# Zolkin1/bilevel-gait-gen

Measured on NVIDIA B200. Metric: A1 SRB-MPC RTI solves/sec, higher is better.
Workload: dtype f64

## Files before the change

bilevel-gait-gen_b200/csrc/bgg_chol.cuh:

```cuda
#pragma once
#include <cuda_runtime.h>

namespace bgg {
namespace chol {

#ifdef BGG_IPM_PROF
static __device__ long long g_chol_prof[16];
#define CPROF_DECL long long cprof_t = clock64();
#define CPROF(k) do { if (threadIdx.x == 0 && blockIdx.x == 0) { const long long t_ = clock64(); g_chol_prof[k] += t_ - cprof_t; cprof_t = t_; } } while (0)
#else
#define CPROF_DECL
#define CPROF(k) do { } while (0)
#endif

__device__ __forceinline__ int blk(int bi, int bj) { return (((bi * (bi + 1)) >> 1) + bj) << 6; }
__device__ __forceinline__ int at(int i, int j) { return blk(i >> 3, j >> 3) + ((i & 7) << 3) + (j & 7); }
__host__ __device__ inline size_t doubles(int nb) { return static_cast<size_t>(nb) * (nb + 1) / 2 * 64; }

__device__ __forceinline__ void dmma(double& c0, double& c1, double a, double b) {
#ifdef BGG_NO_DMMA
    c0 = fma(a, b, c0);
    return;
#endif
    asm volatile("mma.sync.aligned.m8n8k4.row.col.f64.f64.f64.f64 {%0,%1}, {%2}, {%3}, {%0,%1};" : "+d"(c0), "+d"(c1) : "d"(a), "d"(b));
// ... 86 lines not shown
            }
    }
    __syncwarp();
    return bad_any;
}

__device__ __forceinline__ bool factor_invert_diag_v0(double* D, int lane) {
    bool bad_any = false;
    if (lane == 0) {
        double a[8][8];
#pragma unroll
        for (int r = 0; r < 8; ++r)
#pragma unroll
            for (int c = 0; c <= r; ++c) a[r][c] = D[r * 8 + c];
#pragma unroll
        for (int c = 0; c < 8; ++c) {
            const double d = a[c][c];
            const bool bad = !(d > 0.0);
            bad_any |= bad;
            const double inv = bad ? 1.0 : fast_rsqrt(d);
            a[c][c] = inv;
#pragma unroll
            for (int r = c + 1; r < 8; ++r) a[r][c] *= inv;
#pragma unroll
            for (int c2 = c + 1; c2 < 8; ++c2)
#pragma unroll
                for (int r = c2; r < 8; ++r) a[r][c2] -= a[r][c] * a[c2][c];
        }
#pragma unroll
        for (int r = 0; r < 8; ++r)
#pragma unroll
            for (int c = 0; c <= r; ++c) D[r * 8 + c] = a[r][c];
    }
    __syncwarp();
    double x[8];
    if (lane < 8) {
#pragma unroll
        for (int r = 0; r < 8; ++r) {
            double s = 0.0;
#pragma unroll
            for (int k = 0; k < r; ++k) s += D[r * 8 + k] * x[k];
            const double ir = D[r * 8 + r];
            x[r] = (r == lane) ? ir : ((r < lane) ? 0.0 : -ir * s);
        }
    }
    __syncwarp();
    if (lane < 8) {
#pragma unroll
        for (int r = 0; r < 8; ++r) D[r * 8 + lane] = x[r];
    }
    return bad_any;
}

static __device__ __noinline__ void factor(double* K, int nb, int* flag) {
    __builtin_assume(__isShared(K));
    __builtin_assume(__isShared(flag));
    const int tid = threadIdx.x, lane = tid & 31, wid = tid >> 5, nwarp = blockDim.x >> 5;
    if (tid == 0) *flag = 0;
    __syncthreads();
    double2 keep = make_double2(0.0, 0.0);
    CPROF_DECL
    if (wid == 0 && factor_invert_diag(K + blk(0, 0), lane)) *flag = 1;
    __syncthreads();
    const int nother = (nwarp - 1) * 32;
    for (int j = 0; j + 1 < nb; ++j) {
        const double2 X = ldfrag(K + blk(j, j), lane);
        double2 Lj1 = make_double2(0.0, 0.0);
        mma_pqT(Lj1, ldfrag(K + blk(j + 1, j), lane), X);
        if (wid == 0) {
            if (j > 0) stfrag(K + blk(j, j - 1), lane, keep);
            keep = Lj1;
            double2 upd = make_double2(0.0, 0.0);
            mma_pqT(upd, Lj1, Lj1);
            double2 c = ldfrag(K + blk(j + 1, j + 1), lane);
            c.x -= upd.x;
            c.y -= upd.y;
            stfrag(K + blk(j + 1, j + 1), lane, c);
            __syncwarp();
            if (factor_invert_diag(K + blk(j + 1, j + 1), lane)) *flag = 1;
            CPROF(0);
        } else {
            for (int i = j + 2 + (wid - 1); i < nb; i += nwarp - 1) {
                double2 Lij = make_double2(0.0, 0.0);
                mma_pqT(Lij, ldfrag(K + blk(i, j), lane), X);
                stfrag(K + blk(i, j), lane, Lij);
                double2 upd = make_double2(0.0, 0.0);
                mma_pqT(upd, Lij, Lj1);
                double2 c = ldfrag(K + blk(i, j + 1), lane);
                c.x -= upd.x;
                c.y -= upd.y;
                stfrag(K + blk(i, j + 1), lane, c);
            }
            asm volatile("bar.sync 1, %0;" ::"r"(nother) : "memory");
            const int jc = j + 2;
            for (int i = jc + (wid - 1); i < nb; i += nwarp - 1) {
                double2 a0 = make_double2(0.0, 0.0), a1 = make_double2(0.0, 0.0);
                const double* Li = K + blk(i, 0);
                const double* Lj = K + blk(jc, 0);
                int k = 0;
                for (; k + 1 <= j; k += 2) {
                    const double2 p0 = ldfrag(Li + (k << 6), lane), q0 = ldfrag(Lj + (k << 6), lane);
                    const double2 p1 = ldfrag(Li + ((k + 1) << 6), lane), q1 = ldfrag(Lj + ((k + 1) << 6), lane);
                    mma_pqT(a0, p0, q0);
                    mma_pqT(a1, p1, q1);
                }
                if (k <= j) mma_pqT(a0, ldfrag(Li + (k << 6), lane), ldfrag(Lj + (k << 6), lane));
                double2 c = ldfrag(Li + (jc << 6), lane);
                c.x -= a0.x + a1.x;
                c.y -= a0.y + a1.y;
                stfrag(K + blk(i, jc), lane, c);
            }
        }
        __syncthreads();
        CPROF(1);
    }
    if (wid == 0 && nb > 1) stfrag(K + blk(nb - 1, nb - 2), lane, keep);
    __syncthreads();
    CPROF(4);
    for (int h = 1; h <= 4; h <<= 1) {
        const int ngroup = (nb + 2 * h - 1) / (2 * h);
        for (int it = wid; it < ngroup * h; it += nwarp) {
            const int q = it / h, b0 = 2 * h * q, r = b0 + h + it % h;
            if (r >= nb) continue;
            for (int c = b0; c < b0 + h; ++c) {
                double2 T = make_double2(0.0, 0.0);
                for (int k = c; k < b0 + h; ++k) mma_pqT(T, ldfrag(K + blk(r, k), lane), ldfragT(K + blk(k, c), lane));
                __syncwarp();
                stfrag(K + blk(r, c), lane, T);
            }
        }
        __syncthreads();
        for (int it = wid; it < ngroup * h; it += nwarp) {
            const int q = it / h, b0 = 2 * h * q, c = b0 + it % h;
            const int rtop = (b0 + 2 * h < nb) ? b0 + 2 * h : nb;
            for (int r = rtop - 1; r >= b0 + h; --r) {
                double2 Xn = make_double2(0.0, 0.0);
                for (int k = b0 + h; k <= r; ++k) mma_pqT(Xn, ldfrag(K + blk(r, k), lane), ldfragT(K + blk(k, c), lane));
                __syncwarp();
                stfrag(K + blk(r, c), lane, make_double2(-Xn.x, -Xn.y));
                __syncwarp();
            }
        }
        __syncthreads();
    }
    CPROF(5);
}

static __device__ __noinline__ void solve(const double* K, int nb, double* v, double* ys) {
    __builtin_assume(__isShared(K));
    __builtin_assume(__isShared(v));
    __builtin_assume(__isShared(ys));
    const int tid = threadIdx.x, lane = tid & 31, wid = tid >> 5, nwarp = blockDim.x >> 5;
    const int g = lane >> 2, t = lane & 3;
    const int nsup = (nb + 7) >> 3;
    auto row_dot = [&](const double* Kr, const double* x, int qlo, int qhi) -> double {
        double a0 = 0.0, a1 = 0.0;
#pragma unroll 1
        for (int q0 = qlo; q0 < qhi; q0 += 4) {
            double2 p[4], xx[4];
#pragma unroll
            for (int u = 0; u < 4; ++u)
                if (q0 + u < qhi) {
                    p[u] = ldfrag(Kr + ((q0 + u) << 6), lane);
                    xx[u] = *reinterpret_cast<const double2*>(x + 8 * (q0 + u) + 2 * t);
                }
#pragma unroll
            for (int u = 0; u < 4; ++u)
                if (q0 + u < qhi) {
                    a0 = fma(p[u].x, xx[u].x, a0);
                    a1 = fma(p[u].y, xx[u].y, a1);
                }
        }
        a0 += a1;
        a0 += __shfl_xor_sync(0xffffffffu, a0, 1);
        a0 += __shfl_xor_sync(0xffffffffu, a0, 2);
        return a0;
    };
    auto col_dot = [&](int rlo, int rhi, int c, const double* x, int xoff) -> double2 {
        double ax = 0.0, ay = 0.0;
#pragma unroll 1
        for (int r0 = rlo; r0 < rhi; r0 += 4) {
            double2 p[4];
            double xv[4];
#pragma unroll
            for (int u = 0; u < 4; ++u)
                if (r0 + u < rhi) {
                    p[u] = ldfrag(K + blk(r0 + u, c), lane);
                    xv[u] = x[8 * (r0 + u - xoff) + g];
                }
#pragma unroll
            for (int u = 0; u < 4; ++u)
                if (r0 + u < rhi) {
                    ax = fma(p[u].x, xv[u], ax);
                    ay = fma(p[u].y, xv[u], ay);
                }
        }
#pragma unroll
        for (int o = 4; o < 32; o <<= 1) {
            ax += __shfl_xor_sync(0xffffffffu, ax, o);
            ay += __shfl_xor_sync(0xffffffffu, ay, o);
        }
        return make_double2(ax, ay);
    };
    __syncthreads();
    for (int s = 0; s < nsup; ++s) {
        const int b0 = 8 * s, b1 = (b0 + 8 < nb) ? b0 + 8 : nb, cnt = b1 - b0;
        if (wid < cnt) {
            const double a = row_dot(K + blk(b0 + wid, 0), v, b0, b0 + wid + 1);
            if (t == 0) ys[8 * wid + g] = a;
        }
        __syncthreads();
        for (int i = b1 + wid; i < nb; i += nwarp) {
            const double a = row_dot(K + blk(i, 0), ys - 8 * b0, b0, b1);
            if (t == 0) v[8 * i + g] -= a;
        }
        if (tid < 8 * cnt) v[8 * b0 + tid] = ys[tid];
        __syncthreads();
    }
    for (int s = nsup - 1; s >= 0; --s) {
        const int b0 = 8 * s, b1 = (b0 + 8 < nb) ? b0 + 8 : nb, cnt = b1 - b0;
        if (wid < cnt) {
            const double2 a = col_dot(b0 + wid, b1, b0 + wid, v, 0);
            if (g == 0) *reinterpret_cast<double2*>(ys + 8 * wid + 2 * t) = a;
        }
        __syncthreads();
        for (int kb = wid; kb < b0; kb += nwarp) {
            const double2 a = col_dot(b0, b1, kb, ys, b0);
            if (g == 0) {
                double2* dst = reinterpret_cast<double2*>(v + 8 * kb + 2 * t);
                double2 cur = *dst;
                cur.x -= a.x;
                cur.y -= a.y;
                *dst = cur;
            }
        }
        if (tid < 8 * cnt) v[8 * b0 + tid] = ys[tid];
        __syncthreads();
    }
}

}
}
```

bilevel-gait-gen_b200/csrc/bgg_ipm.cu:

```cuda
#include <cstdio>
#include <cstdlib>

#include "bgg_kernels.cuh"
#include "bgg_chol.cuh"
#include "bgg_kkt.cuh"
#include "bgg_kkt_mma.cuh"
#include "bgg_l2ops.cuh"
#ifdef BGG_IPM_TRACE
#include "bgg_ipm_trace.cuh"
#endif

namespace bgg {

#ifdef BGG_IPM_PROF
__device__ long long g_ipm_prof[32];
#define PROF_DECL __shared__ long long s_prof[32]; long long prof_t = 0; if (threadIdx.x == 0) { for (int i_ = 0; i_ < 32; ++i_) s_prof[i_] = 0; prof_t = clock64(); }
#define PROF(k) do { if (threadIdx.x == 0) { const long long t_ = clock64(); s_prof[k] += t_ - prof_t; prof_t = t_; } } while (0)
#define PROF_DUMP do { if (threadIdx.x == 0 && blockIdx.x == 0) for (int i_ = 0; i_ < 32; ++i_) g_ipm_prof[i_] = s_prof[i_]; } while (0)
#else
#define PROF_DECL
#define PROF(k) do { } while (0)
#define PROF_DUMP do { } while (0)
#endif

// ... 55 lines not shown
            fv[cc] = s;
        }
        double* o = out + 6 * j;
        o[0] = fv[2];
        o[1] = -fv[2];
        o[2] = fv[0] - mu_f * fv[2];
        o[3] = -fv[0] - mu_f * fv[2];
        o[4] = fv[1] - mu_f * fv[2];
        o[5] = -fv[1] - mu_f * fv[2];
    }
    if (eout != nullptr && tid >= nth - 32 && tid - (nth - 32) < c.neq) {
        const EqRow& q = c.eq[tid - (nth - 32)];
        double s = -rhs_scale * q.rhs;
        for (int i = 0; i < q.cnt; ++i) s += q.w[i] * v[q.col[i]];
        eout[tid - (nth - 32)] = s;
    }
    __syncthreads();
    #pragma unroll 1
    for (int e = tid; e < ne; e += nth) {
        const int cc = e & 1, foot = (e >> 1) & 3, kk = e >> 3, kf = kk * 4 + foot;
        const double* vv = v + nf + pbase[foot] + cc * npv[foot] + S.poff[kf];
        double s = -S.tkc[kk * 2 + cc];
        for (int i = 0; i < S.pcnt[kf]; ++i) s += S.pw[2 * kf + i] * vv[i];
        out[6 * ns + 2 * e] = s;
        out[6 * ns + 2 * e + 1] = -s;
    }
    __syncthreads();
}

template <bool kRowsShared, int kThreads>
static __device__ __forceinline__ void ipm_add_Ct(const IpmCtx& c, const double* y, double* out, const double* ey, double escale) {
    const Smem S = c.S;
    if (kRowsShared) __builtin_assume(__isShared(y)); __builtin_assume(__isShared(out)); __builtin_assume(__isShared(S.ckc));
    __builtin_assume(__isShared(S.smp)); __builtin_assume(__isShared(S.pw)); __builtin_assume(__isShared(S.col));
    __builtin_assume(__isShared(S.poff));
    const int tid = threadIdx.x;
    constexpr int nth = kThreads;
    const int nu = c.nu, nf = c.nf, ns = c.ns, nkc = c.nkc;
    const double mu_f = c.mu_f;
    #pragma unroll 1
    for (int q = tid; q < nkc; q += nth) {
        const int kk = q >> 1, cc = q & 1;
        double s = 0;
        for (int foot = 0; foot < kNumEE; ++foot) {
            const int e = (kk * 4 + foot) * 2 + cc;
            s += y[6 * ns + 2 * e] - y[6 * ns + 2 * e + 1];
        }
        S.ckc[q] = -s;
    }
    __syncthreads();
    l2_phi_cols_dot(S.phi, S.phi_stride, nkc, nf, smem_addr(S.ckc), smem_addr(out));
    {
        const int half = (2 * nu <= nth) ? 2 : 1;
        #pragma unroll 1
        for (int base = 0; base < half * nu; base += nth) {
            const int it = base + tid;
            const bool act = it < half * nu;
            const int col = act ? it / half : 0, part = it % half;
            const ColInfo ci = S.col[col];
            double s = 0;
            if (!act) {
            } else if (col < nf) {
                if (part == 1 || half == 1)
                    #pragma unroll 1
                    for (int j = ci.lo; j < ci.hi; ++j) {
                        const Sample& sp = S.smp[j];
                        const double* yy = y + 6 * j;
                        double coef;
                        if (ci.coord == 2) coef = (yy[0] - yy[1]) - mu_f * (yy[2] + yy[3] + yy[4] + yy[5]);
                        else if (ci.coord == 0) coef = yy[2] - yy[3];
                        else coef = yy[4] - yy[5];
                        s += coef * sp.w[ci.var - sp.off];
                    }
            } else {
                const int mid = (half == 2) ? (ci.lo + ci.hi + 1) / 2 : ci.hi;
                const int k0 = (part == 0) ? ci.lo : mid, k1 = (part == 0) ? mid : ci.hi;
                #pragma unroll 1
                for (int kk = k0; kk < k1; ++kk) {
                    const int kf = kk * 4 + ci.foot, e = kf * 2 + ci.coord;
                    s += (y[6 * ns + 2 * e] - y[6 * ns + 2 * e + 1]) * S.pw[2 * kf + (ci.var - S.poff[kf])];
                }
                if (ey != nullptr && part == 0) {
                    double se = 0;
                    const int grp = ci.foot * 2 + ci.coord;
                    #pragma unroll 1
                    for (int r = 0; r < c.neq; ++r) {
                        const EqRow& q = c.eq[r];
                        if (q.pad != grp) continue;
                        for (int i = 0; i < q.cnt; ++i)
                            if (q.col[i] == col) se += ey[r] * q.w[i];
                    }
                    s += escale * se;
                }
            }
            if (half == 2) s += __shfl_xor_sync(0xffffffffu, s, 1);
            if (act && part == 0) out[col] += s;
        }
    }
    __syncthreads();
}

static __device__ __forceinline__ void ipm_apply_H(const IpmCtx& c, const double* v, double* out, bool subtract) {
    l2_apply_H(c.Hg, c.nu, smem_addr(v), smem_addr(out), subtract);
}

struct IpmCaps {
// ... 121 lines not shown
        S.poff[i] = nl.poff[foot];
        S.pw[2 * i] = nl.pw[foot][0];
        S.pw[2 * i + 1] = nl.pw[foot][1];
    }
    __shared__ int s_fbase[kNumEE], s_pbase[kNumEE], s_nfv[kNumEE], s_npv[kNumEE];
    __shared__ int s_flag, s_nitems, s_nwork, s_npos;
    __shared__ KktWork s_work[kMaxKktWork];
    __shared__ int s_sb[kNumEE + 1];
    __shared__ EqRow s_eq[kMaxEq];
    if (tid < neq) s_eq[tid] = eqs[tid];
    if (tid < kNumEE) {
        s_fbase[tid] = Hd->fbase[tid];
        s_pbase[tid] = Hd->pbase[tid];
        s_nfv[tid] = Hd->nfv[tid];
        s_npv[tid] = Hd->npv[tid];
    }
    #pragma unroll 1
    for (int i = tid; i < 6 * cap_nu; i += nth) S.u[i] = 0.0;
    if (tid == 0) {
        int e = 0;
        s_sb[0] = 0;
        for (int j = 0; j < ns; ++j)
            while (samples[j].ee > e) s_sb[++e] = j;
        while (e < kNumEE) s_sb[++e] = ns;
    }

    const double box0 = Hd->ee_box[0] / 2, box1 = Hd->ee_box[1] / 2;
    const double fbound = P.force_bound;
    const int m_force = 6 * ns;
    int m_act = 0;
    #pragma unroll 1
    for (int j = tid; j < ns; j += nth) {
        const bool act = samples[j].active != 0;
        for (int r = 0; r < 6; ++r) {
            S.lam[6 * j + r] = act ? 1.0 : 0.0;
            S.s[6 * j + r] = 1.0;
        }
        m_act += act ? 6 : 0;
    }
    #pragma unroll 1
    for (int e = tid; e < ne; e += nth) {
        const int c = e & 1, foot = (e >> 1) & 3, kk = e >> 3;
        const double bx = c ? box1 : box0;
        const double off = xoff[(kk + kEENodeStart) * kNx + c];
        S.d[2 * e + 0] = (bx + P.hip_xy[foot][c]) + off;
        S.d[2 * e + 1] = -(-bx + P.hip_xy[foot][c]) - off;
        S.lam[m_force + 2 * e + 0] = 1.0;
        S.lam[m_force + 2 * e + 1] = 1.0;
        S.s[m_force + 2 * e + 0] = 1.0;
        S.s[m_force + 2 * e + 1] = 1.0;
        m_act += 2;
    }
    auto rhs_of = [&](int i) -> double { return (i < m_force) ? ((i % 6 == 0) ? fbound : 0.0) : S.d[i - m_force]; };
    m_act = static_cast<int>(block_reduce<kSum>(static_cast<double>(m_act), S.red) + 0.5);
    kkt_build_colinfo(S.col, nu, nf, N, s_fbase, s_pbase, s_nfv, s_npv, s_sb, S.smp, S.pcnt, S.poff);
    __syncthreads();
    KktItem* kitems = reinterpret_cast<KktItem*>(ws + L.ktab);
    KktPos* kpos = reinterpret_cast<KktPos*>(ws + L.ktab + sizeof(KktItem) * kMaxKktItems);
    kkt_mma_setup(s_work, &s_nwork, (nu + 7) >> 3, kitems, &s_nitems, s_fbase, s_nfv, S.col, S.smp, kpos, &s_npos, nu, nf, s_eq, neq);
    if (s_nitems > kMaxKktItems || s_npos > kMaxKktPos) {
        if (tid == 0) {
            Hd->status = kOther;
            Hd->no_iterate = 1;
            Hd->iters = 0;
        }
        return;
    }
    __syncthreads();
    PROF(0);
#ifdef BGG_IPM_TRACE
    const trace::Cfg tr_cfg = trace::g_cfg;
    const bool tr_on = tr_cfg.buf != nullptr && tr_cfg.instance == b;
    int tr_n = 0;
    double* tr = nullptr;
    if (tr_on && tid == 0) ++trace::g_cfg.launches;
#endif

    IpmCtx ctx;
    ctx.S = S; ctx.Hg = Hg; ctx.eq = s_eq; ctx.fbase = s_fbase; ctx.pbase = s_pbase; ctx.nfv = s_nfv; ctx.npv = s_npv;
    ctx.N = N; ctx.nu = nu; ctx.nf = nf; ctx.ns = ns; ctx.ne = ne; ctx.neq = neq; ctx.nkc = nkc; ctx.mu_f = mu_f;
    auto apply_C = [&](const double* v, double* out, double* eout, double rhs_scale) { PROF(10); ipm_apply_C<!kSpill, kThreads>(ctx, v, out, eout, rhs_scale); PROF(6); };
    auto add_Ct = [&](const double* y, double* out, const double* ey, double escale) { PROF(10); ipm_add_Ct<!kSpill, kThreads>(ctx, y, out, ey, escale); PROF(7); };
    auto apply_H = [&](const double* v, double* out, bool subtract) { PROF(10); ipm_apply_H(ctx, v, out, subtract); PROF(8); };

    const int nb = (nu + 7) >> 3;
    KktMma km;
    km.K = S.K; km.Hg = Hg; km.phig = phipos; km.phi_ld = L.max_nu; km.nu = nu; km.nf = nf; km.nb = nb; km.ns = ns; km.ne = ne;
    km.neq = neq; km.nkc = nkc; km.wv = S.wv; km.pw = S.pw; km.pcnt = S.pcnt; km.poff = S.poff; km.smp = S.smp; km.eq = s_eq;
    km.col = S.col; km.ckc = S.ckc; km.scratch = S.ds; km.work = s_work; km.nwork = s_nwork; km.items = kitems; km.nitems = s_nitems; km.pos = kpos; km.npos = s_npos;
    km.mu_f = mu_f; km.inv_delta = inv_delta; km.eps = eps;
    auto wrow = [&](int i) -> double {
        const double zi = S.lam[i];
        return (zi > 0.0) ? zi / (S.s[i] + eps * zi) : 0.0;
    };
    auto build_and_factor = [&]() -> bool {
        PROF(10);
        #pragma unroll 1
        for (int i = tid; i < m; i += nth) S.wv[i] = wrow(i);
        __syncthreads();
        kkt_assemble_mma(km);
        PROF(1);
        TRACE(if (tr != nullptr) {
            trace::put_vec(tr, trace::f_w, S.wv, m);
            trace::put_vec(tr, trace::f_K, S.K, static_cast<int>(chol::doubles(nb)));
            __syncthreads();
        });
        chol::factor(S.K, nb, &s_flag);
        PROF(3);
        return s_flag == 0;
    };
    auto solve_K = [&](double* x, bool refine) {
        PROF(10);
        if (refine) {
            #pragma unroll 1
            for (int i = tid; i < nu; i += nth) S.rhs[i] = x[i];
        }
        chol::solve(S.K, nb, x, S.red);
        PROF(5);
        if (refine) {
            #pragma unroll 1
            for (int i = tid; i < nu; i += nth) S.rhs[i] -= eps * x[i];
            __syncthreads();
            apply_H(x, S.rhs, true);
            apply_C(x, S.ds, S.dnu, 0.0);
            #pragma unroll 1
            for (int i = tid; i < m; i += nth) S.ds[i] *= -wrow(i);
            __syncthreads();
            add_Ct(S.ds, S.rhs, S.dnu, -inv_delta);
            PROF(10);
            chol::solve(S.K, nb, S.rhs, S.red);
            PROF(5);
            #pragma unroll 1
            for (int i = tid; i < nu; i += nth) x[i] += S.rhs[i];
            __syncthreads();
        }
    };

    double nrm_q = 1.0, nrm_d = 1.0;
    for (int r = 0; r < kNx; ++r) nrm_q = fmax(nrm_q, fmax(fabs(P.w[r]), fabs(P.Phi_w[r])));
    {
        double v = 0;
        #pragma unroll 1
        for (int i = tid; i < m; i += nth)
            if (S.lam[i] > 0.0) v = fmax(v, fabs(rhs_of(i)));
        for (int r = 0; r < neq; ++r) v = fmax(v, fabs(s_eq[r].rhs));
        nrm_d = fmax(1.0, block_reduce<kMax>(v, S.red));
    }
    if (tid < kMaxEq) S.nueq[tid] = 0.0;
    __syncthreads();

    int it = 0, status = kMaxIter;
    double tau = 1.0, kap = 1.0, mu_first = 0.0;
    double res_p = 0, res_d = 0, gap = 0, gscale = 1, bz = 0, aty_n = 0, zn = 1, pc = 0;
    bool have_point = false;
    int n_refined = 0;
    bool confirm = false;
    for (it = -1; it <= P.ipm_max_iter; ++it) {
        double uHu = 0, rt = 0, mu = 0;
        bool refine_now = false;
        TRACE(if (tr_on) {
            using namespace trace;
            tr = begin_record(tr_cfg, tr_n++);
            put(tr, f_it, it); put(tr, f_threads, kThreads); put(tr, f_spill, kSpill); put(tr, f_stage_phi, stage_phi);
            put(tr, f_cap_nu, cap_nu); put(tr, f_cap_rows, cap_rows); put(tr, f_want, want); put(tr, f_confirm, confirm);
            put(tr, f_N, N); put(tr, f_nu, nu); put(tr, f_nf, nf); put(tr, f_nb, nb); put(tr, f_ns, ns); put(tr, f_ne, ne);
            put(tr, f_m, m); put(tr, f_neq, neq); put(tr, f_m_act, m_act);
            put(tr, f_eps, eps); put(tr, f_delta, delta); put(tr, f_mu_f, mu_f); put(tr, f_tol_feas, P.ipm_tol_feas);
            put(tr, f_tol_gap, P.ipm_tol_gap); put(tr, f_tol_infeas, P.ipm_tol_infeas); put(tr, f_nrm_q, nrm_q);
            put(tr, f_nrm_d, nrm_d); put(tr, f_cost_const, cost_const); put(tr, f_tau, tau); put(tr, f_kap, kap);
            put_vec(tr, f_u, S.u, nu); put_vec(tr, f_s, S.s, m); put_vec(tr, f_z, S.lam, m); put_vec(tr, f_y, S.nueq, neq);
            if (tr != nullptr)
                for (int i = tid; i < m; i += nth) tr[off(f_d) + i] = rhs_of(i);
            __syncthreads();
        });
        if (it >= 0) {
            apply_H(S.u, S.Hu, false);
            #pragma unroll 1
            for (int i = tid; i < nu; i += nth) S.rd[i] = 0.0;
            __syncthreads();
            add_Ct(S.lam, S.rd, S.nueq, 1.0);
            const bool fresh_rz = (it == 0) || confirm;
            if (fresh_rz) apply_C(S.u, S.rp, S.re, tau);
            double r8[8] = {0, 0, 0, 0, 0, 0, 0, 1.0};
            #pragma unroll 1
            for (int i = tid; i < nu; i += nth) {
                const double gi = gg[i], hu = S.Hu[i], ui = S.u[i], at = S.rd[i];
                r8[0] += ui * hu;
                r8[1] += gi * ui;
                r8[4] = fmax(r8[4], fabs(at));
                const double rx = hu + at + gi * tau;
                S.rd[i] = rx;
                r8[5] = fmax(r8[5], fabs(rx));
            }
            #pragma unroll 1
            for (int i = tid; i < m; i += nth) {
                const double zi = S.lam[i];
                if (zi > 0.0) {
                    const double di = rhs_of(i), rz = fresh_rz ? S.rp[i] + S.s[i] - di * tau : S.rp[i];
                    S.rp[i] = rz;
                    r8[2] += di * zi;
                    r8[3] += S.s[i] * zi;
                    r8[6] = fmax(r8[6], fabs(rz));
                    r8[7] = fmax(r8[7], zi);
                } else {
                    S.rp[i] = 0.0;
                }
            }
            PROF(10);
            block_reduce_multi<4, 4>(r8, S.red);
            PROF(13);
            uHu = r8[0];
            const double gu = r8[1];
            double ey = 0, n_re = 0;
            double yn = 0;
            for (int r = 0; r < neq; ++r) {
                ey += s_eq[r].rhs * S.nueq[r];
                n_re = fmax(n_re, fabs(S.re[r]));
                yn = fmax(yn, fabs(S.nueq[r]));
            }
            bz = r8[2] + ey;
            aty_n = r8[4];
            zn = fmax(r8[7], yn);
            rt = kap + gu + bz + uHu / tau;
            mu = (r8[3] + tau * kap) / (m_act + 1);
            pc = (0.5 * uHu / tau + gu) / tau;
            const double dc = (-bz - 0.5 * uHu / tau) / tau;
            const double n_rp = fmax(r8[6], n_re) / tau, n_rd = r8[5] / tau, n_gap = fabs(pc - dc);
            if (!(n_rp == n_rp) || !(n_rd == n_rd) || !(mu == mu) || !(n_gap == n_gap) || !(tau > 0.0)) {
                status = kOther;
                break;
            }
            res_p = n_rp;
            res_d = n_rd;
            gap = n_gap;
            gscale = fmax(1.0, fmin(fabs(pc + cost_const), fabs(dc + cost_const)));
            have_point = true;
            TRACE(if (tr != nullptr) {
                using namespace trace;
                put(tr, f_fresh, fresh_rz); put(tr, f_mu, mu); put(tr, f_rt, rt); put(tr, f_uHu, uHu); put(tr, f_res_p, res_p);
                put(tr, f_res_d, res_d); put(tr, f_gap, gap); put(tr, f_gscale, gscale); put(tr, f_bz, bz); put(tr, f_aty_n, aty_n);
                put(tr, f_zn, zn); put(tr, f_pc, pc);
                put_vec(tr, f_Hu, S.Hu, nu); put_vec(tr, f_rx, S.rd, nu); put_vec(tr, f_rz, S.rp, m); put_vec(tr, f_re, S.re, neq);
                __syncthreads();
            });
            if (res_d <= P.ipm_tol_feas * nrm_q && res_p <= P.ipm_tol_feas * nrm_d && gap <= P.ipm_tol_gap * gscale) {
                if (fresh_rz) {
                    status = kSolved;
                    break;
                }
                confirm = true;
                --it;
                continue;
            }
            confirm = false;
            if (bz < -P.ipm_tol_infeas && aty_n <= P.ipm_tol_infeas * zn * (-bz)) {
                status = kPrimalInfeasible;
                break;
            }
            if (it == P.ipm_max_iter) break;
            if (it == 0) mu_first = mu;
            refine_now = P.ipm_refine > 0 && (mu <= P.ipm_refine_mu_frac * mu_first || it >= P.ipm_refine_from_iter);
            n_refined += refine_now ? 1 : 0;
        }
        if (!build_and_factor()) {
            status = kOther;
            break;
        }
        TRACE(trace::put(tr, trace::f_refine, refine_now););

        double den = 1.0, dtau = 0.0, dkap = 0.0, sigma = 0.0, alpha = 0.0, dkdt_aff = 0.0;
        bool bad = false;
#pragma unroll 1
        for (int pass = 0; pass < (it < 0 ? 1 : 3); ++pass) {
            const double scale = (pass == 0) ? 0.0 : (pass == 1 ? 1.0 : 1.0 - sigma);
            double* x = (pass == 0) ? S.x1 : S.du;
            double* tslot = (pass == 0) ? S.wv : S.ds;
            #pragma unroll 1
            for (int i = tid; i < m; i += nth) {
                const double zi = S.lam[i];
                if (!(zi > 0.0)) {
                    S.ds[i] = 0.0;
                    if (pass > 0) S.dl[i] = 0.0;
                    continue;
                }
                const double w = wrow(i);
                if (pass == 0) {
                    S.ds[i] = w * rhs_of(i);
                } else {
                    double d_s = S.s[i] * zi;
                    if (pass == 2) d_s += S.ds[i] * S.dl[i] - sigma * mu;
                    const double a2 = -scale * S.rp[i] + d_s / zi;
                    S.dl[i] = a2;
                    S.ds[i] = w * a2;
                }
            }
            #pragma unroll 1
            for (int i = tid; i < nu; i += nth) x[i] = (pass == 0) ? -gg[i] : -scale * S.rd[i];
            if (tid < neq) S.a3[tid] = (pass == 0) ? s_eq[tid].rhs : -scale * S.re[tid];
            __syncthreads();
            PROF(14);
            add_Ct(S.ds, x, S.a3, inv_delta);
            solve_K(x, refine_now && pass != 1);
            double* yx = (pass == 0) ? S.y1 : S.dnu;
            apply_C(x, tslot, yx, 0.0);
            if (tid < neq) yx[tid] = (yx[tid] - S.a3[tid]) * inv_delta;
            __syncthreads();
            TRACE(if (tr != nullptr && pass != 1) {
                using namespace trace;
                if (pass == 0) { put_vec(tr, f_x1, S.x1, nu); put_vec(tr, f_cx1, S.wv, m); put_vec(tr, f_y1, S.y1, neq); }
                else { put_vec(tr, f_x2, S.du, nu); put_vec(tr, f_cx2, S.ds, m); put_vec(tr, f_a2, S.dl, m); put_vec(tr, f_y2, S.dnu, neq); }
                __syncthreads();
            });
            if (it < 0) break;
            double r3[3] = {0, 0, 0};
            #pragma unroll 1
            for (int i = tid; i < nu; i += nth) {
                r3[0] += gg[i] * x[i];
                r3[1] += S.Hu[i] * x[i];
            }
            #pragma unroll 1
            for (int i = tid; i < m; i += nth)
                if (S.lam[i] > 0.0) {
                    const double di = rhs_of(i);
                    r3[2] += di * wrow(i) * (tslot[i] - ((pass == 0) ? di : S.dl[i]));
                }
            PROF(10);
            block_reduce_multi<3, 0>(r3, S.red);
            PROF(13);
            double eyx = 0;
            for (int r = 0; r < neq; ++r) eyx += s_eq[r].rhs * yx[r];
            if (pass == 0) {
                den = kap / tau - r3[0] - r3[2] - eyx + uHu / (tau * tau) - 2.0 * r3[1] / tau;
                continue;
            }
            const double d_kap = (pass == 1) ? kap * tau : kap * tau + dkdt_aff - sigma * mu;
            dtau = (scale * rt - d_kap / tau + r3[0] + r3[2] + eyx + 2.0 * r3[1] / tau) / den;
            dkap = (-d_kap - kap * dtau) / tau;
            bool nf_local = !(dtau == dtau) || !(dkap == dkap) || fabs(dtau) > 1e300 || fabs(dkap) > 1e300;
            #pragma unroll 1
            for (int i = tid; i < nu; i += nth) {
                const double v = S.du[i] + dtau * S.x1[i];
                S.du[i] = v;
                nf_local |= !(fabs(v) <= 1e300);
            }
            #pragma unroll 1
            for (int i = tid; i < m; i += nth) {
                const double zi = S.lam[i];
                if (!(zi > 0.0)) continue;
                const double a2 = S.dl[i], di = rhs_of(i);
                const double t = S.ds[i] + dtau * S.wv[i];
                const double dzv = wrow(i) * (t - a2 - dtau * di);
                const double dsv = -(a2 + scale * S.rp[i]) - (S.s[i] / zi) * dzv;
                S.dl[i] = dzv;
                S.ds[i] = dsv;
                if (pass == 2) S.wv[i] = t + dsv - di * dtau;
            }
            if (pass == 2 && tid < neq) S.a3[tid] = delta * S.dnu[tid] + dtau * delta * S.y1[tid] - scale * S.re[tid];
            if (tid < neq) S.dnu[tid] += dtau * S.y1[tid];
            __syncthreads();
            double amax = 1.0;
            #pragma unroll 1
            for (int i = tid; i < m; i += nth) {
                const double zi = S.lam[i];
                if (!(zi > 0.0)) continue;
                const double dsv = S.ds[i], dzv = S.dl[i];
                nf_local |= !(fabs(dzv) <= 1e300) || !(fabs(dsv) <= 1e300);
                if (dsv < 0.0) amax = fmin(amax, -S.s[i] / dsv);
                if (dzv < 0.0) amax = fmin(amax, -zi / dzv);
            }
            PROF(15);
            amax = block_reduce<kMin>(amax, S.red);
            if (__syncthreads_or(nf_local ? 1 : 0)) {
                bad = true;
                break;
            }
            PROF(13);
            if (dtau < 0.0) amax = fmin(amax, -tau / dtau);
            if (dkap < 0.0) amax = fmin(amax, -kap / dkap);
            if (pass == 1) {
                sigma = (1.0 - amax) * (1.0 - amax) * (1.0 - amax);
                dkdt_aff = dkap * dtau;
            } else {
                alpha = 0.99 * amax;
                TRACE(trace::put(tr, trace::f_amax, amax););
            }
        }
        TRACE(if (tr != nullptr && it >= 0 && !bad) {
            using namespace trace;
            put(tr, f_den, den); put(tr, f_sigma, sigma); put(tr, f_dkdt_aff, dkdt_aff); put(tr, f_dtau, dtau); put(tr, f_dkap, dkap);
            put(tr, f_alpha, alpha);
            put_vec(tr, f_du, S.du, nu); put_vec(tr, f_dz, S.dl, m); put_vec(tr, f_ds, S.ds, m); put_vec(tr, f_dy, S.dnu, neq);
            put_vec(tr, f_drz, S.wv, m); put_vec(tr, f_dre, S.a3, neq);
            __syncthreads();
        });
        if (it < 0) {
            double mn[2] = {-1e300, -1e300};
            #pragma unroll 1
            for (int i = tid; i < m; i += nth)
                if (S.lam[i] > 0.0) {
                    const double zv = (S.wv[i] - rhs_of(i)) / (1.0 + eps);
                    S.dl[i] = zv;
                    mn[0] = fmax(mn[0], zv);
                    mn[1] = fmax(mn[1], -zv);
                }
            block_reduce_multi<0, 2>(mn, S.red);
            const double smin = -mn[0], zmin = -mn[1];
            const double sshift = (smin < 1e-8) ? 1.0 - smin : 0.0, zshift = (zmin < 1e-8) ? 1.0 - zmin : 0.0;
            #pragma unroll 1
            for (int i = tid; i < m; i += nth)
                if (S.lam[i] > 0.0) {
                    const double zv = S.dl[i];
                    S.s[i] = -zv + sshift;
                    S.lam[i] = zv + zshift;
                }
            #pragma unroll 1
            for (int i = tid; i < nu; i += nth) S.u[i] = S.x1[i];
            if (tid < neq) S.nueq[tid] = S.y1[tid];
            __syncthreads();
            continue;
        }
        if (bad) {
            status = kOther;
            break;
        }
        #pragma unroll 1
        for (int i = tid; i < nu; i += nth) S.u[i] += alpha * S.du[i];
        #pragma unroll 1
        for (int i = tid; i < m; i += nth)
            if (S.lam[i] > 0.0) {
                S.s[i] += alpha * S.ds[i];
                S.lam[i] += alpha * S.dl[i];
                S.rp[i] += alpha * S.wv[i];
            }
        if (tid < neq) {
            S.nueq[tid] += alpha * S.dnu[tid];
            S.re[tid] += alpha * S.a3[tid];
        }
        tau += alpha * dtau;
        kap += alpha * dkap;
        __syncthreads();
    }
// ... 107 lines not shown
```

bilevel-gait-gen_b200/csrc/bgg_kernels.cuh:

```cuda
#pragma once
#include <cuda_runtime.h>

#include "bgg_spline.cuh"
#include "bgg_types.cuh"
#include "bgg_ws.cuh"

namespace bgg {

__device__ void quat_log3(const double q[4], double out[3]);
__device__ void quat_exp3(const double v[3], double q[4]);
__device__ void quat_first_order_normalize(double q[4]);

__device__ __forceinline__ double warp_sum(double v) {
    for (int o = 16; o > 0; o >>= 1) v += __shfl_xor_sync(0xffffffffu, v, o);
    return v;
}
__device__ __forceinline__ double warp_max(double v) {
    for (int o = 16; o > 0; o >>= 1) v = fmax(v, __shfl_xor_sync(0xffffffffu, v, o));
    return v;
}
__device__ __forceinline__ double warp_min(double v) {
    for (int o = 16; o > 0; o >>= 1) v = fmin(v, __shfl_xor_sync(0xffffffffu, v, o));
    return v;
}
enum RedOp { kSum, kMax, kMin };
template <int OP>
__device__ __noinline__ double block_reduce(double v, double* scratch) {
    const int lane = threadIdx.x & 31, wid = threadIdx.x >> 5, nw = (blockDim.x + 31) >> 5;
    v = (OP == kSum) ? warp_sum(v) : (OP == kMax ? warp_max(v) : warp_min(v));
    __syncthreads();
    if (lane == 0) scratch[wid] = v;
    __syncthreads();
    if (wid == 0) {
        double x = (lane < nw) ? scratch[lane] : ((OP == kSum) ? 0.0 : (OP == kMax ? -1e300 : 1e300));
        x = (OP == kSum) ? warp_sum(x) : (OP == kMax ? warp_max(x) : warp_min(x));
        if (lane == 0) scratch[32] = x;
    }
    __syncthreads();
    return scratch[32];
}

template <int NS, int NM>
__device__ __forceinline__ void block_reduce_multi(double (&v)[NS + NM], double* scratch) {
    const int lane = threadIdx.x & 31, wid = threadIdx.x >> 5, nw = (blockDim.x + 31) >> 5;
#pragma unroll
    for (int k = 0; k < NS + NM; ++k) v[k] = (k < NS) ? warp_sum(v[k]) : warp_max(v[k]);
    __syncthreads();
    if (lane == 0) {
#pragma unroll
        for (int k = 0; k < NS + NM; ++k) scratch[wid * (NS + NM) + k] = v[k];
    }
    __syncthreads();
#pragma unroll
    for (int k = 0; k < NS + NM; ++k) {
        double a = scratch[k];
        for (int w = 1; w < nw; ++w) a = (k < NS) ? a + scratch[w * (NS + NM) + k] : fmax(a, scratch[w * (NS + NM) + k]);
        v[k] = a;
    }
}

void launch_prepare(const Params& P, Instance* inst, const double* state, const double* t0, const double* ee_start,
                    const WsLayout& L, char* ws, int B, cudaStream_t stream);
void launch_ik(const RobotKin& rk, int count, const double* state, const double* ee_des, const double* joint_guess, double* q, int* status,
               int* iters, cudaStream_t stream);
void launch_targets_from_traj(const Params& P, const RobotKin& rk, const Instance* inst, int B, const double* time, double* q_des, double* v_des,
                              double* force_des, int* status, cudaStream_t stream);
constexpr int kPartHdr = 32;
__host__ __device__ size_t param_partials_doubles(int N, int nu_cap);
void launch_param_partials(const Params& P, const Instance* inst, const WsLayout& L, const char* ws, int b, int ee, int idx, int nu_cap, double* out,
                           double* ut, cudaStream_t stream);
void launch_condense(const Params& P, const WsLayout& L, char* ws, int B, int nu_max, int want, cudaStream_t stream);
void launch_ipm(const Params& P, const WsLayout& L, char* ws, int B, int nu_max, int ns_max, int want, cudaStream_t stream, int sm_count = 0);
void launch_batch_max(const WsLayout& L, char* ws, int B, int* out, int cap_nu, int cap_ns, cudaStream_t stream);
size_t finish_smem_bytes(const WsLayout& L);
bool ipm_two_per_sm(const WsLayout& L, int nu_max, int ns_max);
void launch_finish(const Params& P, Instance* inst, const WsLayout& L, char* ws, int B, int want, cudaStream_t stream);
size_t ipm_smem_bytes(const WsLayout& L);
size_t condense_smem_bytes(const WsLayout& L);

void launch_export_dynamics(const Params& P, const WsLayout& L, char* ws, int B, double* Ad, double* Bd, double* cd,
                            int nu_stride, cudaStream_t stream);

void launch_export_csc(const Params& P, const WsLayout& L, const char* ws, int B, int32_t* colptr, int32_t* rowidx, double* val,
                       double* p_diag, double* q, double* ub, int32_t* dims, int n_stride, int m_stride, int nnz_cap,
                       cudaStream_t stream);

int launch_gradient(const Params& P, const Instance* inst, const WsLayout& L, char* ws, int B, int nu_max, int ns_max, int max_smem,
                    cudaStream_t stream);
size_t gradient_smem_bytes(const WsLayout& L, int nu_max, int ns_max);

void launch_gait_lp(const Instance* inst, const WsLayout& L, const char* ws, int B, const double* grad, const double* time, double trust,
                    double alpha, double* step, double* xk, double* times, int32_t* status, cudaStream_t stream);
void launch_ls_expand(const Instance* parent, Instance* child, int B, int K, const double* xk, const double* step, const double* state,
                      const double* t0, const double* ee, double* c_state, double* c_t0, double* c_ee, cudaStream_t stream);
void launch_ls_select(Instance* parent, const Instance* child, const WsLayout& L, const char* child_ws, int B, int K, int32_t* best,
                      double* costs, int32_t* quality, cudaStream_t stream);

}
```

bilevel-gait-gen_b200/csrc/bgg_l2ops.cuh:

```cuda
#pragma once
#include "bgg_kkt_mma.cuh"

namespace bgg {

__device__ __forceinline__ double ldg64(const double* p) {
    double v;
    asm volatile("ld.global.f64 %0, [%1];" : "=d"(v) : "l"(p));
    return v;
}
__device__ __forceinline__ double ldany64(const double* p) {
    double v;
    asm volatile("ld.f64 %0, [%1];" : "=d"(v) : "l"(p));
    return v;
}

static __device__ __noinline__ void l2_apply_H(const double* __restrict__ Hg, int nu, unsigned v_s, unsigned out_s, bool subtract) {
    const int tid = threadIdx.x, nth = blockDim.x;
    const int half = (2 * nu <= nth) ? 2 : 1;
    for (int base = 0; base < half * nu; base += nth) {
        const int it = base + tid;
        const bool act = it < half * nu;
        const int part = (act && it >= nu && half == 2) ? 1 : 0, i = act ? it - part * nu : 0;
        const int j0 = (half == 2) ? (part * nu) / 2 : 0, j1 = (half == 2) ? ((part + 1) * nu) / 2 : nu;
        double s0 = 0.0, s1 = 0.0;
        if (act) {
            const double* col = Hg + i;
            for (int jb = j0; jb < j1; jb += 20) {
                double hv[20];
#pragma unroll
                for (int k = 0; k < 20; ++k) hv[k] = ldg64(col + static_cast<size_t>(min(jb + k, j1 - 1)) * nu);
#pragma unroll
                for (int k = 0; k < 20; k += 2) {
                    if (jb + k < j1) s0 = fma(hv[k], lds64(v_s + 8u * (jb + k)), s0);
                    if (jb + k + 1 < j1) s1 = fma(hv[k + 1], lds64(v_s + 8u * (jb + k + 1)), s1);
                }
            }
        }
        const double s = subtract ? -(s0 + s1) : s0 + s1;
        if (half == 2) {
            if (act && part == 1) sts64(out_s + 8u * i, subtract ? lds64(out_s + 8u * i) + s : s);
            __syncthreads();
            if (act && part == 0) sts64(out_s + 8u * i, lds64(out_s + 8u * i) + s);
        } else if (act) {
            sts64(out_s + 8u * i, subtract ? lds64(out_s + 8u * i) + s : s);
        }
    }
    __syncthreads();
}

static __device__ __noinline__ void l2_phi_rows_dot(const double* __restrict__ phi, int stride, int nkc, int nf, unsigned v_s, unsigned tkc_s) {
    const int tid = threadIdx.x, lane = tid & 31, wid = tid >> 5, nwarp = blockDim.x >> 5;
    double vv[5];
#pragma unroll
    for (int k = 0; k < 5; ++k) vv[k] = (lane + 32 * k < nf) ? lds64(v_s + 8u * (lane + 32 * k)) : 0.0;
    for (int q0 = wid; q0 < nkc; q0 += 5 * nwarp) {
        double part[5];
#pragma unroll
        for (int r = 0; r < 5; ++r) {
            const int q = q0 + r * nwarp;
            double ph[5];
#pragma unroll
            for (int k = 0; k < 5; ++k) ph[k] = (q < nkc && lane + 32 * k < nf) ? phi[static_cast<size_t>(q) * stride + lane + 32 * k] : 0.0;
            double sacc = 0.0;
#pragma unroll
            for (int k = 0; k < 5; ++k) sacc = fma(ph[k], vv[k], sacc);
            part[r] = sacc;
        }
#pragma unroll
        for (int o = 16; o > 0; o >>= 1) {
#pragma unroll
            for (int r = 0; r < 5; ++r) part[r] += __shfl_xor_sync(0xffffffffu, part[r], o);
        }
#pragma unroll
        for (int r = 0; r < 5; ++r) {
            const int q = q0 + r * nwarp;
            if (lane == 0 && q < nkc) sts64(tkc_s + 8u * q, part[r]);
        }
    }
}

static __device__ __noinline__ void l2_phi_cols_dot(const double* __restrict__ phi, int stride, int nkc, int nf, unsigned ckc_s, unsigned out_s) {
    const int tid = threadIdx.x, nth = blockDim.x;
    for (int base = 0; base < 2 * nf; base += nth) {
        const int it = base + tid;
        const bool act = it < 2 * nf;
        const int col = act ? it >> 1 : 0, part = it & 1;
        const int qh = (nkc + 1) >> 1, q0 = part ? qh : 0, q1 = part ? nkc : qh;
        double s0 = 0.0, s1 = 0.0;
        if (act) {
            const double* pc = phi + col;
            for (int qb = q0; qb < q1; qb += 24) {
                double ph[24];
#pragma unroll
                for (int k = 0; k < 24; ++k) ph[k] = ldany64(pc + static_cast<size_t>(min(qb + k, q1 - 1)) * stride);
#pragma unroll
                for (int k = 0; k < 24; k += 2) {
                    if (qb + k < q1) s0 = fma(lds64(ckc_s + 8u * (qb + k)), ph[k], s0);
                    if (qb + k + 1 < q1) s1 = fma(lds64(ckc_s + 8u * (qb + k + 1)), ph[k + 1], s1);
                }
            }
        }
        double s = s0 + s1;
        s += __shfl_xor_sync(0xffffffffu, s, 1);
        if (act && part == 0) sts64(out_s + 8u * col, lds64(out_s + 8u * col) + s);
    }
    __syncthreads();
}

}
```

Before: 117,800.

## Interleave blocked triangular inverse steps into Cholesky factor loop

Moves the recursive-doubling inversion of the lower-triangular Cholesky factor out of a separate post-pass and schedules each group's steps as soon as their source blocks are final, running them on the non-diagonal warps inside the factor loop. The aim is to overlap inversion work with the serial diagonal chain handled by warp 0 and to remove several full-block barriers at the end. It also hoists a diagonal-block load ahead of the store in warp 0. The trade-off is more complex index logic, extra named-barrier syncs per iteration, and a risk of ordering bugs if the readiness conditions are wrong.

```diff
diff --git a/bilevel-gait-gen_b200/csrc/bgg_chol.cuh b/bilevel-gait-gen_b200/csrc/bgg_chol.cuh
--- a/bilevel-gait-gen_b200/csrc/bgg_chol.cuh
+++ b/bilevel-gait-gen_b200/csrc/bgg_chol.cuh
@@ -162,6 +162,49 @@
     return bad_any;
 }
 
+__device__ __forceinline__ int inv_last(int h, int b0, int nb) { return (b0 + 2 * h < nb ? b0 + 2 * h : nb) - 1; }
+__device__ __forceinline__ int inv_stepA(int h, int b0, int nb) { const int b1 = inv_last(h, b0, nb); return b0 + h + 1 > b1 - 1 ? b0 + h + 1 : b1 - 1; }
+__device__ __forceinline__ int inv_stepB(int h, int b0, int nb) { return inv_last(h, b0, nb) + 1; }
+
+template <typename Sync>
+__device__ __forceinline__ void invert_step(double* K, int nb, int s, int w, int nw, int lane, Sync sync) {
+    int n = 0;
+    for (int h = 1; h <= 4; h <<= 1)
+        for (int b0 = 0; b0 + h < nb; b0 += 2 * h) {
+            if (inv_stepA(h, b0, nb) != s) continue;
+            const int b1 = inv_last(h, b0, nb);
+            for (int r = b0 + h; r <= b1; ++r, ++n) {
+                if (n % nw != w) continue;
+                for (int c = b0; c < b0 + h; ++c) {
+                    double2 T = make_double2(0.0, 0.0);
+                    for (int k = c; k < b0 + h; ++k) mma_pqT(T, ldfrag(K + blk(r, k), lane), ldfragT(K + blk(k, c), lane));
+                    __syncwarp();
+                    stfrag(K + blk(r, c), lane, T);
+                }
+            }
+        }
+    bool pending = n > 0;
+    for (int h = 1; h <= 4; h <<= 1) {
+        n = 0;
+        for (int b0 = 0; b0 + h < nb; b0 += 2 * h) {
+            if (inv_stepB(h, b0, nb) != s) continue;
+            if (n == 0 && pending) sync();
+            const int b1 = inv_last(h, b0, nb);
+            for (int c = b0; c < b0 + h; ++c, ++n) {
+                if (n % nw != w) continue;
+                for (int r = b1; r >= b0 + h; --r) {
+                    double2 Xn = make_double2(0.0, 0.0);
+                    for (int k = b0 + h; k <= r; ++k) mma_pqT(Xn, ldfrag(K + blk(r, k), lane), ldfragT(K + blk(k, c), lane));
+                    __syncwarp();
+                    stfrag(K + blk(r, c), lane, make_double2(-Xn.x, -Xn.y));
+                    __syncwarp();
+                }
+            }
+        }
+        pending |= n > 0;
+    }
+}
+
 static __device__ __noinline__ void factor(double* K, int nb, int* flag) {
     __builtin_assume(__isShared(K));
     __builtin_assume(__isShared(flag));
@@ -173,16 +216,17 @@
     if (wid == 0 && factor_invert_diag(K + blk(0, 0), lane)) *flag = 1;
     __syncthreads();
     const int nother = (nwarp - 1) * 32;
+    const auto bar_others = [nother]() { asm volatile("bar.sync 1, %0;" ::"r"(nother) : "memory"); };
     for (int j = 0; j + 1 < nb; ++j) {
         const double2 X = ldfrag(K + blk(j, j), lane);
         double2 Lj1 = make_double2(0.0, 0.0);
         mma_pqT(Lj1, ldfrag(K + blk(j + 1, j), lane), X);
         if (wid == 0) {
+            double2 c = ldfrag(K + blk(j + 1, j + 1), lane);
             if (j > 0) stfrag(K + blk(j, j - 1), lane, keep);
             keep = Lj1;
             double2 upd = make_double2(0.0, 0.0);
             mma_pqT(upd, Lj1, Lj1);
-            double2 c = ldfrag(K + blk(j + 1, j + 1), lane);
             c.x -= upd.x;
             c.y -= upd.y;
             stfrag(K + blk(j + 1, j + 1), lane, c);
@@ -201,7 +245,7 @@
                 c.y -= upd.y;
                 stfrag(K + blk(i, j + 1), lane, c);
             }
-            asm volatile("bar.sync 1, %0;" ::"r"(nother) : "memory");
+            bar_others();
             const int jc = j + 2;
             for (int i = jc + (wid - 1); i < nb; i += nwarp - 1) {
                 double2 a0 = make_double2(0.0, 0.0), a1 = make_double2(0.0, 0.0);
@@ -220,6 +264,7 @@
                 c.y -= a0.y + a1.y;
                 stfrag(K + blk(i, jc), lane, c);
             }
+            invert_step(K, nb, j, wid - 1, nwarp - 1, lane, bar_others);
         }
         __syncthreads();
         CPROF(1);
@@ -227,32 +272,11 @@
     if (wid == 0 && nb > 1) stfrag(K + blk(nb - 1, nb - 2), lane, keep);
     __syncthreads();
     CPROF(4);
-    for (int h = 1; h <= 4; h <<= 1) {
-        const int ngroup = (nb + 2 * h - 1) / (2 * h);
-        for (int it = wid; it < ngroup * h; it += nwarp) {
-            const int q = it / h, b0 = 2 * h * q, r = b0 + h + it % h;
-            if (r >= nb) continue;
-            for (int c = b0; c < b0 + h; ++c) {
-                double2 T = make_double2(0.0, 0.0);
-                for (int k = c; k < b0 + h; ++k) mma_pqT(T, ldfrag(K + blk(r, k), lane), ldfragT(K + blk(k, c), lane));
-                __syncwarp();
-                stfrag(K + blk(r, c), lane, T);
-            }
-        }
-        __syncthreads();
-        for (int it = wid; it < ngroup * h; it += nwarp) {
-            const int q = it / h, b0 = 2 * h * q, c = b0 + it % h;
-            const int rtop = (b0 + 2 * h < nb) ? b0 + 2 * h : nb;
-            for (int r = rtop - 1; r >= b0 + h; --r) {
-                double2 Xn = make_double2(0.0, 0.0);
-                for (int k = b0 + h; k <= r; ++k) mma_pqT(Xn, ldfrag(K + blk(r, k), lane), ldfragT(K + blk(k, c), lane));
-                __syncwarp();
-                stfrag(K + blk(r, c), lane, make_double2(-Xn.x, -Xn.y));
-                __syncwarp();
-            }
-        }
-        __syncthreads();
-    }
+    const auto bar_all = []() { __syncthreads(); };
+    invert_step(K, nb, nb - 1, wid, nwarp, lane, bar_all);
+    __syncthreads();
+    invert_step(K, nb, nb, wid, nwarp, lane, bar_all);
+    __syncthreads();
     CPROF(5);
 }
 
```

Result: slower. 92740, median of 6 (-21.3%).

## Remove redundant block barriers and fuse step-length reductions in IPM iteration

Applied to the files above, without the earlier changes.

Drops several __syncthreads calls at function boundaries and in the reductions, relying on barriers that callers already place (a 'fenced' reduce variant). block_reduce now broadcasts the result through all warps instead of a second barrier round, and the min step length plus the non-finite flag are merged into one multi-reduction. The dual-variable update is deferred until after the loop. The goal is fewer block-wide barriers per IPM iteration in a latency-bound single-block solver. In exchange it risks shared-memory races if any of the removed barriers was actually needed.

```diff
diff --git a/bilevel-gait-gen_b200/csrc/bgg_chol.cuh b/bilevel-gait-gen_b200/csrc/bgg_chol.cuh
--- a/bilevel-gait-gen_b200/csrc/bgg_chol.cuh
+++ b/bilevel-gait-gen_b200/csrc/bgg_chol.cuh
@@ -312,7 +312,6 @@
         }
         return make_double2(ax, ay);
     };
-    __syncthreads();
     for (int s = 0; s < nsup; ++s) {
         const int b0 = 8 * s, b1 = (b0 + 8 < nb) ? b0 + 8 : nb, cnt = b1 - b0;
         if (wid < cnt) {
diff --git a/bilevel-gait-gen_b200/csrc/bgg_ipm.cu b/bilevel-gait-gen_b200/csrc/bgg_ipm.cu
--- a/bilevel-gait-gen_b200/csrc/bgg_ipm.cu
+++ b/bilevel-gait-gen_b200/csrc/bgg_ipm.cu
@@ -131,6 +131,7 @@
     l2_phi_cols_dot(S.phi, S.phi_stride, nkc, nf, smem_addr(S.ckc), smem_addr(out));
     {
         const int half = (2 * nu <= nth) ? 2 : 1;
+        if (half == 1) __syncthreads();
         #pragma unroll 1
         for (int base = 0; base < half * nu; base += nth) {
             const int it = base + tid;
@@ -358,7 +359,7 @@
         m_act += 2;
     }
     auto rhs_of = [&](int i) -> double { return (i < m_force) ? ((i % 6 == 0) ? fbound : 0.0) : S.d[i - m_force]; };
-    m_act = static_cast<int>(block_reduce<kSum>(static_cast<double>(m_act), S.red) + 0.5);
+    m_act = static_cast<int>(block_reduce<kSum, true>(static_cast<double>(m_act), S.red) + 0.5);
     kkt_build_colinfo(S.col, nu, nf, N, s_fbase, s_pbase, s_nfv, s_npv, s_sb, S.smp, S.pcnt, S.poff);
     __syncthreads();
     KktItem* kitems = reinterpret_cast<KktItem*>(ws + L.ktab);
@@ -450,7 +451,7 @@
         for (int i = tid; i < m; i += nth)
             if (S.lam[i] > 0.0) v = fmax(v, fabs(rhs_of(i)));
         for (int r = 0; r < neq; ++r) v = fmax(v, fabs(s_eq[r].rhs));
-        nrm_d = fmax(1.0, block_reduce<kMax>(v, S.red));
+        nrm_d = fmax(1.0, block_reduce<kMax, true>(v, S.red));
     }
     if (tid < kMaxEq) S.nueq[tid] = 0.0;
     __syncthreads();
@@ -483,7 +484,6 @@
             apply_H(S.u, S.Hu, false);
             #pragma unroll 1
             for (int i = tid; i < nu; i += nth) S.rd[i] = 0.0;
-            __syncthreads();
             add_Ct(S.lam, S.rd, S.nueq, 1.0);
             const bool fresh_rz = (it == 0) || confirm;
             if (fresh_rz) apply_C(S.u, S.rp, S.re, tau);
@@ -513,7 +513,7 @@
                 }
             }
             PROF(10);
-            block_reduce_multi<4, 4>(r8, S.red);
+            block_reduce_multi<4, 4, true>(r8, S.red);
             PROF(13);
             uHu = r8[0];
             const double gu = r8[1];
@@ -610,9 +610,9 @@
             double* yx = (pass == 0) ? S.y1 : S.dnu;
             apply_C(x, tslot, yx, 0.0);
             if (tid < neq) yx[tid] = (yx[tid] - S.a3[tid]) * inv_delta;
-            __syncthreads();
             TRACE(if (tr != nullptr && pass != 1) {
                 using namespace trace;
+                __syncthreads();
                 if (pass == 0) { put_vec(tr, f_x1, S.x1, nu); put_vec(tr, f_cx1, S.wv, m); put_vec(tr, f_y1, S.y1, neq); }
                 else { put_vec(tr, f_x2, S.du, nu); put_vec(tr, f_cx2, S.ds, m); put_vec(tr, f_a2, S.dl, m); put_vec(tr, f_y2, S.dnu, neq); }
                 __syncthreads();
@@ -631,7 +631,7 @@
                     r3[2] += di * wrow(i) * (tslot[i] - ((pass == 0) ? di : S.dl[i]));
                 }
             PROF(10);
-            block_reduce_multi<3, 0>(r3, S.red);
+            block_reduce_multi<3, 0, true>(r3, S.red);
             PROF(13);
             double eyx = 0;
             for (int r = 0; r < neq; ++r) eyx += s_eq[r].rhs * yx[r];
@@ -642,6 +642,7 @@
             const double d_kap = (pass == 1) ? kap * tau : kap * tau + dkdt_aff - sigma * mu;
             dtau = (scale * rt - d_kap / tau + r3[0] + r3[2] + eyx + 2.0 * r3[1] / tau) / den;
             dkap = (-d_kap - kap * dtau) / tau;
+            double amax = 1.0;
             bool nf_local = !(dtau == dtau) || !(dkap == dkap) || fabs(dtau) > 1e300 || fabs(dkap) > 1e300;
             #pragma unroll 1
             for (int i = tid; i < nu; i += nth) {
@@ -660,26 +661,18 @@
                 S.dl[i] = dzv;
                 S.ds[i] = dsv;
                 if (pass == 2) S.wv[i] = t + dsv - di * dtau;
-            }
-            if (pass == 2 && tid < neq) S.a3[tid] = delta * S.dnu[tid] + dtau * delta * S.y1[tid] - scale * S.re[tid];
-            if (tid < neq) S.dnu[tid] += dtau * S.y1[tid];
-            __syncthreads();
-            double amax = 1.0;
-            #pragma unroll 1
-            for (int i = tid; i < m; i += nth) {
-                const double zi = S.lam[i];
-                if (!(zi > 0.0)) continue;
-                const double dsv = S.ds[i], dzv = S.dl[i];
                 nf_local |= !(fabs(dzv) <= 1e300) || !(fabs(dsv) <= 1e300);
                 if (dsv < 0.0) amax = fmin(amax, -S.s[i] / dsv);
                 if (dzv < 0.0) amax = fmin(amax, -zi / dzv);
             }
             PROF(15);
-            amax = block_reduce<kMin>(amax, S.red);
-            if (__syncthreads_or(nf_local ? 1 : 0)) {
+            double mx[2] = {-amax, nf_local ? 1.0 : 0.0};
+            block_reduce_multi<0, 2, true>(mx, S.red + 3 * (nth / 32));
+            if (mx[1] > 0.0) {
                 bad = true;
                 break;
             }
+            amax = -mx[0];
             PROF(13);
             if (dtau < 0.0) amax = fmin(amax, -tau / dtau);
             if (dkap < 0.0) amax = fmin(amax, -kap / dkap);
@@ -691,8 +684,14 @@
                 TRACE(trace::put(tr, trace::f_amax, amax););
             }
         }
+        if (it >= 0 && !bad && tid < neq) {
+            const double scale = 1.0 - sigma;
+            S.a3[tid] = delta * S.dnu[tid] + dtau * delta * S.y1[tid] - scale * S.re[tid];
+            S.dnu[tid] += dtau * S.y1[tid];
+        }
         TRACE(if (tr != nullptr && it >= 0 && !bad) {
             using namespace trace;
+            __syncthreads();
             put(tr, f_den, den); put(tr, f_sigma, sigma); put(tr, f_dkdt_aff, dkdt_aff); put(tr, f_dtau, dtau); put(tr, f_dkap, dkap);
             put(tr, f_alpha, alpha);
             put_vec(tr, f_du, S.du, nu); put_vec(tr, f_dz, S.dl, m); put_vec(tr, f_ds, S.ds, m); put_vec(tr, f_dy, S.dnu, neq);
diff --git a/bilevel-gait-gen_b200/csrc/bgg_kernels.cuh b/bilevel-gait-gen_b200/csrc/bgg_kernels.cuh
--- a/bilevel-gait-gen_b200/csrc/bgg_kernels.cuh
+++ b/bilevel-gait-gen_b200/csrc/bgg_kernels.cuh
@@ -24,28 +24,23 @@
     return v;
 }
 enum RedOp { kSum, kMax, kMin };
-template <int OP>
+template <int OP, bool kFenced = false>
 __device__ __noinline__ double block_reduce(double v, double* scratch) {
     const int lane = threadIdx.x & 31, wid = threadIdx.x >> 5, nw = (blockDim.x + 31) >> 5;
     v = (OP == kSum) ? warp_sum(v) : (OP == kMax ? warp_max(v) : warp_min(v));
-    __syncthreads();
+    if (!kFenced) __syncthreads();
     if (lane == 0) scratch[wid] = v;
     __syncthreads();
-    if (wid == 0) {
-        double x = (lane < nw) ? scratch[lane] : ((OP == kSum) ? 0.0 : (OP == kMax ? -1e300 : 1e300));
-        x = (OP == kSum) ? warp_sum(x) : (OP == kMax ? warp_max(x) : warp_min(x));
-        if (lane == 0) scratch[32] = x;
-    }
-    __syncthreads();
-    return scratch[32];
+    double x = (lane < nw) ? scratch[lane] : ((OP == kSum) ? 0.0 : (OP == kMax ? -1e300 : 1e300));
+    return (OP == kSum) ? warp_sum(x) : (OP == kMax ? warp_max(x) : warp_min(x));
 }
 
-template <int NS, int NM>
+template <int NS, int NM, bool kFenced = false>
 __device__ __forceinline__ void block_reduce_multi(double (&v)[NS + NM], double* scratch) {
     const int lane = threadIdx.x & 31, wid = threadIdx.x >> 5, nw = (blockDim.x + 31) >> 5;
 #pragma unroll
     for (int k = 0; k < NS + NM; ++k) v[k] = (k < NS) ? warp_sum(v[k]) : warp_max(v[k]);
-    __syncthreads();
+    if (!kFenced) __syncthreads();
     if (lane == 0) {
 #pragma unroll
         for (int k = 0; k < NS + NM; ++k) scratch[wid * (NS + NM) + k] = v[k];
diff --git a/bilevel-gait-gen_b200/csrc/bgg_l2ops.cuh b/bilevel-gait-gen_b200/csrc/bgg_l2ops.cuh
--- a/bilevel-gait-gen_b200/csrc/bgg_l2ops.cuh
+++ b/bilevel-gait-gen_b200/csrc/bgg_l2ops.cuh
@@ -45,7 +45,6 @@
             sts64(out_s + 8u * i, subtract ? lds64(out_s + 8u * i) + s : s);
         }
     }
-    __syncthreads();
 }
 
 static __device__ __noinline__ void l2_phi_rows_dot(const double* __restrict__ phi, int stride, int nkc, int nf, unsigned v_s, unsigned tkc_s) {
@@ -104,7 +103,6 @@
         s += __shfl_xor_sync(0xffffffffu, s, 1);
         if (act && part == 0) sts64(out_s + 8u * col, lds64(out_s + 8u * col) + s);
     }
-    __syncthreads();
 }
 
 }
```

After: 117,600 before, 117,400 after (median of 6 runs). Within noise of the previous version (-0.2%).
